# deevinandu/Distributed-Multi-Agent-SLAM-Swarm-Robotics-System

Measured on NVIDIA B200. Metric: beam_cell_updates_per_sec, higher is better.
Workload: dtype f64+u32

## Files before the change

### distributed-multi-agent-slam-swarm-robotics-system_b200/csrc/occgrid_tiled.cu

```cuda
#include "common.cuh"

namespace occ {

constexpr int kTT = 256;
constexpr int kChunkPk = 2048;
constexpr int kChunkMin = 256;
constexpr int kItemsPerCta = 3;
constexpr int kMaxWindowBytes = 100 * 1024;

struct TilePlanHeader {
    unsigned int n_items, n_active, total_records, work_counter, resolve_counter, overflow;
    unsigned int active_count;
    unsigned int pad;
};

__device__ __forceinline__ int home_tile(const Geom& g, const TileGeom& tg, double rx, double ry) {
    const double qx = cell_quotient(rx, g.ox, g.res), qy = cell_quotient(ry, g.oy, g.res);
    if (!quotient_in_range(qx) || !quotient_in_range(qy)) return -1;
    const int px = trunc_cell(qx) - g.win_x0 + tg.pad, py = trunc_cell(qy) - g.win_y0 + tg.pad;
    if (px < tg.pad - tg.reach || py < tg.pad - tg.reach || px >= tg.pad + g.win_w + tg.reach ||
        py >= tg.pad + g.win_h + tg.reach)
        return -1;
    return (py >> kTileShift) * tg.tiles_x + (px >> kTileShift);
}

constexpr int kPkPerCta = 2048;
constexpr int kSub = kPkPerCta / kTT;
constexpr int kHash = 4096;
constexpr unsigned int kEmpty = 0xffffffffu;
static_assert(kHash >= 2 * kPkPerCta, "hash table must stay at most half full");

__device__ __forceinline__ int hash_insert(unsigned int* keys, unsigned int tile) {
    unsigned int h = (tile * 2654435761u) >> 20;
    for (;;) {
        const unsigned int old = atomicCAS(&keys[h], kEmpty, tile);
        if (old == kEmpty || old == tile) return (int)h;
        h = (h + 1) & (kHash - 1);
    }
}

constexpr int kHashPerThread = kHash / kTT;

__device__ __forceinline__ void flush_tile_counts(const unsigned int* s_keys, const unsigned int* s_vals,
                                                  unsigned int* __restrict__ tile_count, unsigned int* __restrict__ active,
                                                  TilePlanHeader* __restrict__ hdr) {
    unsigned int key[kHashPerThread], old[kHashPerThread];
#pragma unroll
    for (int j = 0; j < kHashPerThread; ++j) {
        const int i = j * kTT + threadIdx.x;
        key[j] = s_keys[i];
        old[j] = 1u;
        if (key[j] != kEmpty) old[j] = atomicAdd(&tile_count[key[j]], s_vals[i]);
    }
#pragma unroll
    for (int j = 0; j < kHashPerThread; ++j)
        if (key[j] != kEmpty && old[j] == 0u) active[atomicAdd(&hdr->active_count, 1u)] = key[j];
}

__device__ __forceinline__ void reserve_tile_ranges(const unsigned int* s_keys, unsigned int* s_vals,
                                                    const unsigned int* __restrict__ tile_offset, unsigned int* __restrict__ tile_cursor) {
    unsigned int key[kHashPerThread], base[kHashPerThread], off[kHashPerThread];
#pragma unroll
    for (int j = 0; j < kHashPerThread; ++j) {
        const int i = j * kTT + threadIdx.x;
        key[j] = s_keys[i];
        base[j] = off[j] = 0u;
        if (key[j] != kEmpty) { off[j] = tile_offset[key[j]]; base[j] = atomicAdd(&tile_cursor[key[j]], s_vals[i]); }
    }
#pragma unroll
    for (int j = 0; j < kHashPerThread; ++j)
        if (key[j] != kEmpty) s_vals[j * kTT + threadIdx.x] = off[j] + base[j];
}

constexpr size_t kBinSmem = (size_t)kTT * kMaxRecStride + 2 * kHash * sizeof(unsigned int) + kPkPerCta * sizeof(unsigned short);
constexpr unsigned int kNoSlot = 0xffffu;

template <bool kMaps = false>
__global__ void __launch_bounds__(kTT)
k_home_bin(Geom g, TileGeom tg, const uint8_t* __restrict__ pkts, long long n, int stride,
           const int32_t* __restrict__ agent_idx, const double* __restrict__ drift,
           const double* __restrict__ agent_off, int n_agents,
           unsigned int* __restrict__ tile_count, PoseRec* __restrict__ recs, unsigned int* __restrict__ local_bins, uint2* __restrict__ runs,
           unsigned int* __restrict__ seg_count, unsigned int* __restrict__ active, TilePlanHeader* __restrict__ hdr,
           uint64_t* counters) {
    extern __shared__ __align__(16) uint8_t s_bin[];
    uint8_t* const s_rec = s_bin;
    unsigned int* const s_keys = reinterpret_cast<unsigned int*>(s_bin + kTT * kMaxRecStride);
    unsigned int* const s_vals = s_keys + kHash;
    unsigned short* const s_slot = reinterpret_cast<unsigned short*>(s_vals + kHash);
    __shared__ unsigned int s_wsum[kTT / 32];
    for (int i = threadIdx.x; i < kHash; i += kTT) { s_keys[i] = kEmpty; s_vals[i] = 0u; }
    unsigned long long c[OCCGRID_C_HITS + 1] = {};
    const long long cta_first = (long long)blockIdx.x * kPkPerCta;
    constexpr int kVec = (kTT * kMaxRecStride / 16 + kTT - 1) / kTT;
    uint4 pre[kVec];
    auto prefetch = [&](int sub) {
        const long long first = cta_first + (long long)sub * kTT;
        const long long left = n - first;
        const size_t bytes = left <= 0 ? 0 : (size_t)min((long long)kTT, left) * stride;
        const uint4* s4 = reinterpret_cast<const uint4*>(pkts + (size_t)first * stride);
#pragma unroll
        for (int j = 0; j < kVec; ++j) {
            const size_t i = (size_t)j * kTT + threadIdx.x;
            pre[j] = (i * 16 + 16 <= bytes) ? __ldg(s4 + i) : make_uint4(0u, 0u, 0u, 0u);
        }
    };
    const bool vec_ok = (reinterpret_cast<uintptr_t>(pkts) & 15) == 0 && ((kTT * stride) & 15) == 0;
    if (vec_ok) prefetch(0);
    for (int sub = 0; sub < kSub; ++sub) {
        const long long first = cta_first + (long long)sub * kTT;
        if (first >= n) break;
        const int count = (int)min((long long)kTT, n - first);
        __syncthreads();
        if (vec_ok) {
            const size_t bytes = (size_t)count * stride;
            uint4* d4 = reinterpret_cast<uint4*>(s_rec);
#pragma unroll
            for (int j = 0; j < kVec; ++j) {
                const size_t i = (size_t)j * kTT + threadIdx.x;
                if (i * 16 + 16 <= bytes) d4[i] = pre[j];
            }
            for (size_t i = (bytes / 16) * 16 + threadIdx.x; i < bytes; i += kTT) s_rec[i] = __ldg(pkts + (size_t)first * stride + i);
            if (sub + 1 < kSub) prefetch(sub + 1);
        } else {
            stage_records(pkts + (size_t)first * stride, (size_t)count * stride, s_rec);
        }
        __syncthreads();
        if ((int)threadIdx.x < count) {
            const long long k = first + threadIdx.x;
            double rx, ry, ryaw;
            float dist[4];
            c[OCCGRID_C_PACKETS] += 1;
            unsigned int slot = kNoSlot;
            int agent = 1;
            const int st = decode_packet(s_rec + threadIdx.x * stride, k, agent_idx, drift, agent_off, n_agents, &rx, &ry, &ryaw, dist,
                                         kMaps ? &agent : nullptr);
            if (st == PKT_DROPPED) c[OCCGRID_C_DROPPED] += 1;
            else if (st == PKT_BAD_POSE) c[OCCGRID_C_BAD_POSE] += 1;
            else {
                c[OCCGRID_C_ACCEPTED] += 1;
                c[OCCGRID_C_BEAMS] += 4;
#pragma unroll
                for (int s = 0; s < 4; ++s) {
                    const double d = (double)dist[s];
                    c[OCCGRID_C_HITS] += (OCC_MIN_DIST_M < d && d <= OCC_MAX_DIST_M) ? 1 : 0;
                }
                int tile = home_tile(g, tg, rx, ry);
                if (kMaps && tile >= 0) tile += (agent - 1) * tg.n_tiles;
                if (tile >= 0) {
                    slot = (unsigned int)hash_insert(s_keys, (unsigned int)tile);
                    atomicAdd(&s_vals[slot], 1u);
                    PoseRec r;
                    r.rx = rx; r.ry = ry; r.yaw = (float)ryaw;
                    r.d[0] = dist[0]; r.d[1] = dist[1]; r.d[2] = dist[2]; r.d[3] = dist[3];
                    r.k = (unsigned int)k;
                    r.tile = tile; r.pad = 0;
                    recs[k] = r;
                }
            }
            s_slot[sub * kTT + threadIdx.x] = (unsigned short)slot;
        }
    }
    __syncthreads();
    unsigned int key[kHashPerThread], rank[kHashPerThread];
#pragma unroll
    for (int j = 0; j < kHashPerThread; ++j) {
        const int i = j * kTT + threadIdx.x;
        key[j] = s_keys[i];
        rank[j] = 0u;
        if (key[j] != kEmpty) rank[j] = atomicAdd(&tile_count[key[j]], s_vals[i]);
    }
    const int lane = threadIdx.x & 31, warp = threadIdx.x >> 5;
    unsigned int mine = 0u;
#pragma unroll
    for (int j = 0; j < kHashPerThread; ++j) mine += key[j] != kEmpty ? s_vals[j * kTT + threadIdx.x] + 0x10000u : 0u;
    unsigned int inc = mine;
#pragma unroll
    for (int o = 1; o < 32; o <<= 1) { const unsigned int u = __shfl_up_sync(0xffffffffu, inc, o); if (lane >= o) inc += u; }
    if (lane == 31) s_wsum[warp] = inc;
    __syncthreads();
    unsigned int pos = inc - mine, n_local = 0u;
#pragma unroll
    for (int w = 0; w < kTT / 32; ++w) {
        pos += w < warp ? s_wsum[w] : 0u;
        n_local += s_wsum[w];
    }
    n_local &= 0xffffu;
    if (threadIdx.x == 0) seg_count[blockIdx.x] = n_local;
    const size_t seg0 = (size_t)blockIdx.x * kPkPerCta;
#pragma unroll
    for (int j = 0; j < kHashPerThread; ++j) {
        if (key[j] == kEmpty) continue;
        const int i = j * kTT + threadIdx.x;
        const unsigned int run = pos >> 16, begin = pos & 0xffffu;
        runs[seg0 + run] = make_uint2(key[j], rank[j] - begin);
        pos += s_vals[i] + 0x10000u;
        s_keys[i] = run;
        s_vals[i] = begin;
        if (rank[j] == 0u) active[atomicAdd(&hdr->active_count, 1u)] = key[j];
    }
    __syncthreads();
    unsigned int* const s_local = reinterpret_cast<unsigned int*>(s_rec);
    const int n_seg = (int)min((long long)kPkPerCta, n - (long long)seg0);
    for (int j = threadIdx.x; j < n_seg; j += kTT) {
        const unsigned int slot = s_slot[j];
        if (slot != kNoSlot) s_local[atomicAdd(&s_vals[slot], 1u)] = (s_keys[slot] << 16) | (unsigned int)j;
    }
    __syncthreads();
    for (unsigned int j = threadIdx.x; j < n_local; j += kTT) local_bins[seg0 + j] = s_local[j];
    __syncthreads();
    block_add_counters(c, reinterpret_cast<unsigned long long*>(s_rec), counters);
}

__global__ void __launch_bounds__(kTT)
k_place_runs(const unsigned int* __restrict__ local_bins, const uint2* __restrict__ runs, const unsigned int* __restrict__ seg_count,
             const unsigned int* __restrict__ tile_offset, const TilePlanHeader* __restrict__ hdr, unsigned int* __restrict__ bins) {
    if (hdr->overflow) return;
    const size_t seg0 = (size_t)blockIdx.x * kPkPerCta;
    const int n_local = (int)seg_count[blockIdx.x];
    unsigned int e[kSub], off[kSub];
    uint2 d[kSub];
#pragma unroll
    for (int sub = 0; sub < kSub; ++sub) {
        const int j = sub * kTT + threadIdx.x;
        e[sub] = j < n_local ? local_bins[seg0 + j] : kEmpty;
    }
#pragma unroll
    for (int sub = 0; sub < kSub; ++sub) d[sub] = e[sub] != kEmpty ? runs[seg0 + (e[sub] >> 16)] : make_uint2(0u, 0u);
#pragma unroll
    for (int sub = 0; sub < kSub; ++sub) off[sub] = e[sub] != kEmpty ? tile_offset[d[sub].x] : 0u;
#pragma unroll
    for (int sub = 0; sub < kSub; ++sub)
        if (e[sub] != kEmpty) bins[off[sub] + d[sub].y + (unsigned int)(sub * kTT + threadIdx.x)] = (unsigned int)(seg0 + (e[sub] & 0xffffu));
}

__device__ __forceinline__ int chunk_valid(const SegInfo& seg, long long chunk, long long* addr0) {
    const long long a0 = chunk * kSegChunk;
    *addr0 = a0;
    const unsigned int sg = (unsigned int)(a0 / seg.seg_cap);
    const unsigned int j0 = (unsigned int)(a0 - (long long)sg * seg.seg_cap);
    unsigned int cnt = seg.d_counts ? seg.d_counts[sg] : seg.host_count;
    if (cnt > seg.seg_cap) cnt = seg.seg_cap;
    return cnt > j0 ? (int)min((unsigned int)kSegChunk, cnt - j0) : 0;
}

__global__ void __launch_bounds__(kTT)
k_home_count_poses(Geom g, TileGeom tg, const PoseRec* __restrict__ recs, const int* __restrict__ in_tiles, SegInfo seg, long long n_chunks,
                   int tiles_in_records,
                   unsigned int* __restrict__ tile_count, int* __restrict__ tile_ids,
                   unsigned int* __restrict__ active, TilePlanHeader* __restrict__ hdr, uint64_t* counters) {
    __shared__ unsigned int s_keys[kHash];
    __shared__ unsigned int s_vals[kHash];
    __shared__ unsigned long long s_acc[(OCCGRID_C_HITS + 1) * 32];
    unsigned long long c[OCCGRID_C_HITS + 1] = {};
    for (long long chunk = blockIdx.x; chunk < n_chunks; chunk += gridDim.x) {
        long long addr0;
        const int valid = chunk_valid(seg, chunk, &addr0);
        if (valid == 0) continue;
        for (int i = threadIdx.x; i < kHash; i += kTT) { s_keys[i] = kEmpty; s_vals[i] = 0u; }
        __syncthreads();
        if (tiles_in_records) {
            int tl[kSub];
#pragma unroll
            for (int sub = 0; sub < kSub; ++sub) {
                const int j = sub * kTT + threadIdx.x;
                tl[sub] = -1;
                if (j < valid) tl[sub] = in_tiles ? in_tiles[addr0 + j] : recs[addr0 + j].tile;
            }
#pragma unroll
            for (int sub = 0; sub < kSub; ++sub) {
                const int j = sub * kTT + threadIdx.x;
                if (j >= valid) continue;
                int tile = tl[sub];
                if (tile >= tg.n_tiles) tile = -1;
                if (tile >= 0) atomicAdd(&s_vals[hash_insert(s_keys, (unsigned int)tile)], 1u);
                tile_ids[addr0 + j] = tile;
            }
        } else {
            for (int sub = 0; sub < kSub; ++sub) {
                const int j = sub * kTT + threadIdx.x;
                if (j >= valid) break;
                const long long k = addr0 + j;
                int tile = -1;
                const PoseRec r = recs[k];
                c[OCCGRID_C_PACKETS] += 1;
                if (!(isfinite(r.rx) && isfinite(r.ry) && isfinite(r.yaw))) c[OCCGRID_C_BAD_POSE] += 1;
                else {
                    c[OCCGRID_C_ACCEPTED] += 1;
                    c[OCCGRID_C_BEAMS] += 4;
#pragma unroll
                    for (int s2 = 0; s2 < 4; ++s2) {
                        const double dd = (double)r.d[s2];
                        c[OCCGRID_C_HITS] += (OCC_MIN_DIST_M < dd && dd <= OCC_MAX_DIST_M) ? 1 : 0;
                    }
                    tile = home_tile(g, tg, r.rx, r.ry);
                }
                if (tile >= 0) atomicAdd(&s_vals[hash_insert(s_keys, (unsigned int)tile)], 1u);
                tile_ids[k] = tile;
            }
        }
        __syncthreads();
        flush_tile_counts(s_keys, s_vals, tile_count, active, hdr);
        __syncthreads();
    }
    block_add_counters(c, s_acc, counters);
}

__global__ void __launch_bounds__(kTT)
k_home_scatter_segs(SegInfo seg, long long n_chunks, const int* __restrict__ tile_ids, const unsigned int* __restrict__ tile_offset,
                    unsigned int* __restrict__ tile_cursor, const TilePlanHeader* __restrict__ hdr, unsigned int* __restrict__ bins) {
    __shared__ unsigned int s_keys[kHash];
    __shared__ unsigned int s_vals[kHash];
    if (hdr->overflow) return;
    for (long long chunk = blockIdx.x; chunk < n_chunks; chunk += gridDim.x) {
        long long addr0;
        const int valid = chunk_valid(seg, chunk, &addr0);
        if (valid == 0) continue;
        for (int i = threadIdx.x; i < kHash; i += kTT) { s_keys[i] = kEmpty; s_vals[i] = 0u; }
        __syncthreads();
        unsigned int where[kSub];
        int tl[kSub];
#pragma unroll
        for (int sub = 0; sub < kSub; ++sub) {
            const int j = sub * kTT + threadIdx.x;
            tl[sub] = j < valid ? tile_ids[addr0 + j] : -1;
        }
#pragma unroll
        for (int sub = 0; sub < kSub; ++sub) {
            const int j = sub * kTT + threadIdx.x;
            where[sub] = kEmpty;
            if (j < valid) {
                const int tile = tl[sub];
                if (tile >= 0) {
                    const int h = hash_insert(s_keys, (unsigned int)tile);
                    where[sub] = ((unsigned int)h << 16) | atomicAdd(&s_vals[h], 1u);
                }
            }
        }
        __syncthreads();
        reserve_tile_ranges(s_keys, s_vals, tile_offset, tile_cursor);
        __syncthreads();
#pragma unroll
        for (int sub = 0; sub < kSub; ++sub)
            if (where[sub] != kEmpty)
                bins[s_vals[where[sub] >> 16] + (where[sub] & 0xffffu)] = (unsigned int)(addr0 + sub * kTT + threadIdx.x);
        __syncthreads();
    }
}

__global__ void __launch_bounds__(1024)
k_tile_plan(unsigned int* __restrict__ tile_count, unsigned int* __restrict__ tile_offset,
            unsigned int* __restrict__ tile_cursor, uint4* __restrict__ items, unsigned int max_items,
            const unsigned int* __restrict__ active, unsigned long long max_records, TilePlanHeader* __restrict__ hdr,
            uint64_t* counters, unsigned int target_items) {
    __shared__ unsigned int s_warp[2][33];
    __shared__ unsigned int s_carry[2];
    __shared__ unsigned int s_total;
    if (threadIdx.x < 2) s_carry[threadIdx.x] = 0;
    if (threadIdx.x == 0) s_total = 0;
    __syncthreads();
    const int n_active = (int)hdr->active_count;
    const int lane = threadIdx.x & 31, warp = threadIdx.x >> 5;
    {
        unsigned int mine = 0;
        for (int i = threadIdx.x; i < n_active; i += blockDim.x) mine += tile_count[active[i]];
#pragma unroll
        for (int o = 16; o > 0; o >>= 1) mine += __shfl_xor_sync(0xffffffffu, mine, o);
        if (lane == 0 && mine) atomicAdd(&s_total, mine);
    }
    __syncthreads();
    unsigned int chunk_pk = (s_total / target_items + kChunkMin) / kChunkMin * kChunkMin;
    chunk_pk = chunk_pk > (unsigned int)kChunkPk ? (unsigned int)kChunkPk : chunk_pk;
    for (int start = 0; start < n_active; start += blockDim.x) {
        const int i = start + threadIdx.x;
        const unsigned int t = i < n_active ? active[i] : 0u;
        const unsigned int cnt = i < n_active ? tile_count[t] : 0u;
        unsigned int v[2] = {cnt, (cnt + chunk_pk - 1) / chunk_pk};
        unsigned int ex[2];
#pragma unroll
        for (int j = 0; j < 2; ++j) {
            unsigned int inc = v[j];
#pragma unroll
            for (int o = 1; o < 32; o <<= 1) { unsigned int u = __shfl_up_sync(0xffffffffu, inc, o); if (lane >= o) inc += u; }
            if (lane == 31) s_warp[j][warp] = inc;
            ex[j] = inc - v[j];
        }
        __syncthreads();
        if (warp < 2) {
            unsigned int w = s_warp[warp][lane], winc = w;
#pragma unroll
            for (int o = 1; o < 32; o <<= 1) { unsigned int u = __shfl_up_sync(0xffffffffu, winc, o); if (lane >= o) winc += u; }
            s_warp[warp][lane] = winc - w;
            if (lane == 31) s_warp[warp][32] = winc;
        }
        __syncthreads();
        const unsigned int off = s_carry[0] + s_warp[0][warp] + ex[0];
        const unsigned int item0 = s_carry[1] + s_warp[1][warp] + ex[1];
        if (i < n_active) {
            tile_offset[t] = off;
            tile_cursor[t] = 0u;
            tile_count[t] = 0u;
            for (unsigned int j = 0; j < v[1]; ++j) {
                const unsigned int b = off + j * chunk_pk;
                const unsigned int e = min(off + cnt, b + chunk_pk);
                if (item0 + j < max_items) items[item0 + j] = make_uint4(t, b, e, 0u);
            }
        }
        __syncthreads();
        if (threadIdx.x < 2) s_carry[threadIdx.x] += s_warp[threadIdx.x][32];
        __syncthreads();
    }
    if (threadIdx.x == 0) {
        TilePlanHeader h;
        h.total_records = s_carry[0];
        h.n_items = s_carry[1];
        h.n_active = (unsigned int)n_active;
        h.work_counter = 0;
        h.resolve_counter = 0;
        h.active_count = 0;
        h.overflow = (s_carry[0] > max_records || s_carry[1] > max_items) ? 1u : 0u;
        if (h.overflow) { h.n_items = 0; h.n_active = 0; }
        h.pad = 0;
        *hdr = h;
        if (counters) atomicAdd(reinterpret_cast<unsigned long long*>(counters) + OCCGRID_C_RECORDS, (unsigned long long)s_carry[0]);
    }
}

__device__ __noinline__ void draw_beam_smem(unsigned int* __restrict__ s_win, int side, int pitch, int x, int y,
                                               int ddx, int ddy, unsigned int free_stamp, bool hit, bool skip_first) {
    const int dx = abs(ddx), dy = abs(ddy);
    int err = dx - dy;
    const int n = max(dx, dy);
    const unsigned int us = (unsigned int)side;
    if ((unsigned int)x < us && (unsigned int)y < us && (unsigned int)(x + ddx) < us && (unsigned int)(y + ddy) < us) {
        const int sxo = ddx > 0 ? 1 : -1;
        const int syo = ddy > 0 ? pitch : -pitch;
        const bool xmajor = dx >= dy;
        const int dmaj = xmajor ? dx : dy, dmin = xmajor ? dy : dx;
        const int step_maj = xmajor ? sxo : syo;
        const int step_both = sxo + syo;
        const int e_minor = dmaj - dmin;
        int E = dmaj - dmin;
        int off = y * pitch + x;
        int i = 0;
        if (skip_first) {
            if (n == 0) return;
            const bool minor = 2 * E < dmaj;
            off += minor ? step_both : step_maj;
            E += minor ? e_minor : -dmin;
            i = 1;
        }
        for (; i < n; ++i) {
            atomicMax(&s_win[off], free_stamp);
            const bool minor = 2 * E < dmaj;
            off += minor ? step_both : step_maj;
            E += minor ? e_minor : -dmin;
        }
        if (hit) atomicMax(&s_win[off], free_stamp | 1u);
        return;
    }
    const int sx = ddx > 0 ? 1 : -1, sy = ddy > 0 ? 1 : -1;
    for (int i = 0; i < n; ++i) {
        if (!(i == 0 && skip_first) && (unsigned int)x < us && (unsigned int)y < us) atomicMax(&s_win[y * pitch + x], free_stamp);
        const int e2 = 2 * err;
        if (e2 > -dy) { err -= dy; x += sx; }
        if (e2 < dx)  { err += dx; y += sy; }
    }
    if (hit && !(n == 0 && skip_first) && (unsigned int)x < us && (unsigned int)y < us) atomicMax(&s_win[y * pitch + x], free_stamp | 1u);
}

__device__ __noinline__ void count_beam_smem(unsigned int* __restrict__ s_win, int side, int pitch, int x, int y,
                                                int ddx, int ddy, bool hit) {
    const int dx = abs(ddx), dy = abs(ddy);
    const int n = max(dx, dy);
    const unsigned int us = (unsigned int)side;
    if ((unsigned int)x < us && (unsigned int)y < us && (unsigned int)(x + ddx) < us && (unsigned int)(y + ddy) < us) {
        const int sxo = ddx > 0 ? 1 : -1;
        const int syo = ddy > 0 ? pitch : -pitch;
        const bool xmajor = dx >= dy;
        const int dmaj = xmajor ? dx : dy, dmin = xmajor ? dy : dx;
        const int step_maj = xmajor ? sxo : syo;
        const int step_both = sxo + syo;
        const int e_minor = dmaj - dmin;
        int E = dmaj - dmin;
        int off = y * pitch + x;
        for (int i = 0; i < n; ++i) {
            atomicAdd(&s_win[off], 1u);
            const bool minor = 2 * E < dmaj;
            off += minor ? step_both : step_maj;
            E += minor ? e_minor : -dmin;
        }
        if (hit) atomicAdd(&s_win[off], 0x10000u);
        return;
    }
    int err = dx - dy;
    const int sx = ddx > 0 ? 1 : -1, sy = ddy > 0 ? 1 : -1;
    for (int i = 0; i < n; ++i) {
        if ((unsigned int)x < us && (unsigned int)y < us) atomicAdd(&s_win[y * pitch + x], 1u);
        const int e2 = 2 * err;
        if (e2 > -dy) { err -= dy; x += sx; }
        if (e2 < dx)  { err += dx; y += sy; }
    }
    if (hit && (unsigned int)x < us && (unsigned int)y < us) atomicAdd(&s_win[y * pitch + x], 0x10000u);
}



constexpr int kMaskMaxLen = 32;
constexpr int kMaskEntries = (kMaskMaxLen + 1) * (kMaskMaxLen + 2) / 2;

__device__ __forceinline__ unsigned int walk_mask_of(int dmaj, int dmin) {
    unsigned int m = 0u;
    int E = dmaj - dmin;
    for (int i = 0; i < dmaj; ++i) {
        const bool minor = 2 * E < dmaj;
        m |= (minor ? 1u : 0u) << i;
        E += minor ? (dmaj - dmin) : -dmin;
    }
    return m;
}

__device__ __forceinline__ void build_walk_masks(unsigned int* s_mask) {
    for (int e = threadIdx.x; e < kMaskEntries; e += blockDim.x) {
        int dmaj = 0;
        while ((dmaj + 1) * (dmaj + 2) / 2 <= e) ++dmaj;
        s_mask[e] = walk_mask_of(dmaj, e - dmaj * (dmaj + 1) / 2);
    }
}

template <bool kAdd>
__device__ __forceinline__ void smem_red(unsigned int addr, unsigned int v) {
    if (kAdd) asm volatile("red.shared.add.u32 [%0], %1;" ::"r"(addr), "r"(v) : "memory");
    else      asm volatile("red.shared.max.u32 [%0], %1;" ::"r"(addr), "r"(v) : "memory");
}

template <bool kAdd>
__device__ __forceinline__ void walk_beam_masked(unsigned int win, int pitch, int x, int y, int ddx, int ddy,
                                                 unsigned int v_free, bool hit, bool skip_first, const unsigned int* s_mask) {
    const int dx = abs(ddx), dy = abs(ddy);
    const bool xmajor = dx >= dy;
    const int dmaj = xmajor ? dx : dy, dmin = xmajor ? dy : dx;
    const int sx4 = ddx > 0 ? 4 : -4;
    const int sy4 = (ddy > 0 ? pitch : -pitch) * 4;
    const int step_maj = xmajor ? sx4 : sy4, step_min = xmajor ? sy4 : sx4;
    unsigned int mask = s_mask[dmaj * (dmaj + 1) / 2 + dmin];
    unsigned int a = win + (unsigned int)(y * pitch + x) * 4u;
    const unsigned int a_end = a + (unsigned int)((ddy * pitch + ddx) * 4);
    int rem = dmaj;
    if (rem > 0) {
        if (!skip_first) smem_red<kAdd>(a, v_free);
        a += step_maj + ((mask & 1u) ? step_min : 0);
        mask >>= 1;
        --rem;
    }
    while (rem >= 8) {
#pragma unroll
        for (int j = 0; j < 8; ++j) {
            smem_red<kAdd>(a, v_free);
            a += step_maj + ((mask & (1u << j)) ? step_min : 0);
        }
        mask >>= 8;
        rem -= 8;
    }
    if (rem >= 4) {
#pragma unroll
        for (int j = 0; j < 4; ++j) {
            smem_red<kAdd>(a, v_free);
            a += step_maj + ((mask & (1u << j)) ? step_min : 0);
        }
        mask >>= 4;
        rem -= 4;
    }
    for (; rem > 0; --rem) {
        smem_red<kAdd>(a, v_free);
        a += step_maj + ((mask & 1u) ? step_min : 0);
        mask >>= 1;
    }
// ... 395 lines not shown
        for (int ly = ly_lo + part * (kTT / 32) + warp; ly < ly_hi; ly += kResolveSplit * (kTT / 32)) {
            const size_t row = (size_t)(wy0 + ly) * g.win_w + wx0;
            for (int lx = lx_lo + lane; lx < lx_hi; lx += 32) {
                const unsigned int s = plane[row + lx];
                if (s) {
                    map_grid[row + lx] = (s & 1u) ? OCCGRID_CELL_OCCUPIED : OCCGRID_CELL_FREE;
                    plane[row + lx] = 0u;
                }
            }
        }
    }
}


static int g_raycast_cta_cap = 0;
void set_raycast_cta_cap(int cap) { g_raycast_cta_cap = cap < 0 ? 0 : cap; }

struct TiledLayout {
    size_t off_stamps, off_count, off_offset, off_cursor, off_active, off_hdr, off_items, off_ids, off_bins, off_local, off_runs,
        off_segs, off_recs, total;
    unsigned long long max_records;
    unsigned int max_items;
};

static TiledLayout tiled_layout(const occgrid_geom* geom, int64_t max_records, bool packets, int n_maps = 1) {
    TiledLayout L;
    const TileGeom tg = tile_geom(geom);
    const size_t n_keys = (size_t)n_maps * tg.n_tiles;
    L.max_records = (unsigned long long)max_records;
    unsigned long long items = L.max_records / kChunkMin + (unsigned long long)n_keys + 1;
    if (items > L.max_records + 1) items = L.max_records + 1;
    L.max_items = (unsigned int)items;
    size_t o = 0;
    L.off_stamps = o; o += align_up((size_t)geom->win_w * geom->win_h * 4 * (size_t)n_maps, 256);
    L.off_count = o;  o += align_up((n_keys + 1) * 4, 256);
    L.off_offset = o; o += align_up((n_keys + 1) * 4, 256);
    L.off_cursor = o; o += align_up((n_keys + 1) * 4, 256);
    L.off_active = o; o += align_up((n_keys + 1) * 4, 256);
    L.off_hdr = o;    o += 256;
    L.off_items = o;  o += align_up((size_t)L.max_items * sizeof(uint4), 256);
    L.off_ids = o;    o += packets ? 0 : align_up((size_t)L.max_records * sizeof(int), 256);
    L.off_bins = o;   o += align_up((size_t)L.max_records * sizeof(unsigned int), 256);
    L.off_local = o;  o += packets ? align_up((size_t)L.max_records * sizeof(unsigned int), 256) : 0;
    L.off_runs = o;   o += packets ? align_up((size_t)L.max_records * sizeof(uint2), 256) : 0;
    L.off_segs = o;   o += packets ? align_up((size_t)(L.max_records + kPkPerCta - 1) / kPkPerCta * sizeof(unsigned int), 256) : 0;
    L.off_recs = o;   o += packets ? align_up((size_t)L.max_records * sizeof(PoseRec), 256) : 0;
    L.total = o;
    return L;
}

bool tiled_supported(const occgrid_geom* geom, int n_maps) {
    const TileGeom tg = tile_geom(geom);
    return (size_t)tg.win_side * tg.pitch * 4 <= (size_t)kMaxWindowBytes && (long long)n_maps * tg.n_tiles <= (1ll << 24);
}

size_t tiled_workspace_bytes(const occgrid_geom* geom, int n_maps, int64_t max_packets) {
    return tiled_layout(geom, max_packets < 1 ? 1 : max_packets, true, n_maps).total;
}

size_t tiled_band_workspace_bytes(const occgrid_geom* geom, int n_segs, int64_t seg_cap) {
    return tiled_layout(geom, (int64_t)n_segs * seg_cap, false).total;
}

struct TiledPtrs {
    unsigned int *stamps, *tile_count, *tile_offset, *tile_cursor, *active, *bins, *local_bins, *seg_count;
    TilePlanHeader* hdr;
    uint4* items;
    int* tile_ids;
    uint2* runs;
    PoseRec* recs;
};

static TiledPtrs tiled_ptrs(const TiledLayout& L, void* d_ws) {
    char* ws = reinterpret_cast<char*>(d_ws);
    TiledPtrs p;
    p.stamps = reinterpret_cast<unsigned int*>(ws + L.off_stamps);
    p.tile_count = reinterpret_cast<unsigned int*>(ws + L.off_count);
    p.tile_offset = reinterpret_cast<unsigned int*>(ws + L.off_offset);
    p.tile_cursor = reinterpret_cast<unsigned int*>(ws + L.off_cursor);
    p.active = reinterpret_cast<unsigned int*>(ws + L.off_active);
    p.hdr = reinterpret_cast<TilePlanHeader*>(ws + L.off_hdr);
    p.items = reinterpret_cast<uint4*>(ws + L.off_items);
    p.bins = reinterpret_cast<unsigned int*>(ws + L.off_bins);
    p.tile_ids = reinterpret_cast<int*>(ws + L.off_ids);
    p.local_bins = reinterpret_cast<unsigned int*>(ws + L.off_local);
    p.runs = reinterpret_cast<uint2*>(ws + L.off_runs);
    p.seg_count = reinterpret_cast<unsigned int*>(ws + L.off_segs);
    p.recs = reinterpret_cast<PoseRec*>(ws + L.off_recs);
    return p;
}

static size_t raycast_smem(const TileGeom& tg, bool route) {
    size_t b = (size_t)tg.win_side * tg.pitch * 4;
    const size_t r = (size_t)kRouteItemPk * 2 * sizeof(PoseRec);
    const size_t raw = (size_t)kRouteItemPk * kMaxRecStride;
    if (route) b = b > r ? b : r;
    if (route) b = b > raw ? b : raw;
    return b;
}

template <bool kCounts, bool kRoute, bool kMaps = false>
static int launch_raycast(const Geom& g, const TileGeom& tg, const TiledPtrs& P, const PoseRec* recs, int ordinals_in_records,
                          unsigned int* plane, uint64_t* d_counters, int have_items, const RouteJob& job, cudaStream_t st) {
    const size_t smem = raycast_smem(tg, kRoute);
    static thread_local size_t configured = 0;
    if (smem > configured) {
        OCC_CUDA_TRY(cudaFuncSetAttribute(k_home_raycast<kCounts, kRoute, kMaps>, cudaFuncAttributeMaxDynamicSharedMemorySize, (int)smem));
        configured = smem;
    }
    int ctas_per_sm = 1;
    if (cudaOccupancyMaxActiveBlocksPerMultiprocessor(&ctas_per_sm, k_home_raycast<kCounts, kRoute, kMaps>, kTT, smem) != cudaSuccess || ctas_per_sm < 1)
        ctas_per_sm = 1;
    if (g_raycast_cta_cap > 0 && ctas_per_sm > g_raycast_cta_cap) ctas_per_sm = g_raycast_cta_cap;
    ProfileScope ps(K_TILE_RAYCAST, st);
    k_home_raycast<kCounts, kRoute, kMaps><<<device_sm_count() * ctas_per_sm, kTT, smem, st>>>(g, tg, P.items, P.hdr, P.bins, recs,
                                                                                               ordinals_in_records, plane, d_counters,
                                                                                               have_items, job);
    return OCCGRID_OK;
}

static unsigned int plan_target_items() { return (unsigned int)device_sm_count() * 3u * (unsigned int)kItemsPerCta; }

static int grid_chunks(long long n_chunks) {
    long long b = n_chunks < 1 ? 1 : n_chunks;
    const long long cap = (long long)device_sm_count() * 8;
    return (int)(b < cap ? b : cap);
}

int integrate_tiled(const occgrid_geom* geom, const PacketBatch& batch, const PoseRec* d_poses, int ordinals_in_records, Output kind,
                    void* d_out, void* d_ws, size_t ws_bytes, uint64_t* d_counters, cudaStream_t st) {
    const int64_t n = batch.n;
    const bool maps = kind == Output::kAgentMaps;
    const TiledLayout L = tiled_layout(geom, n, d_poses == nullptr, maps ? batch.n_agents : 1);
    if (ws_bytes < L.total) {
        set_last_error("workspace %zu B < %zu B needed by TILED for %lld records", ws_bytes, L.total, (long long)n);
        return OCCGRID_E_WORKSPACE;
    }
    const TiledPtrs P = tiled_ptrs(L, d_ws);
    const PoseRec* recs = d_poses ? d_poses : P.recs;
    const Geom g = to_geom(geom);
    const TileGeom tg = tile_geom(geom);
    const unsigned int blocks = (unsigned int)((n + kPkPerCta - 1) / kPkPerCta);
    SegInfo seg;
    seg.n_segs = 1; seg.seg_cap = (unsigned int)align_up((size_t)n, kSegChunk); seg.d_counts = nullptr; seg.host_count = (unsigned int)n;
    const long long n_chunks = (n + kSegChunk - 1) / kSegChunk;
    {
        ProfileScope ps(K_TILE_COUNT, st);
        if (d_poses) {
            k_home_count_poses<<<grid_chunks(n_chunks), kTT, 0, st>>>(g, tg, d_poses, nullptr, seg, n_chunks, 0, P.tile_count, P.tile_ids, P.active,
                                                                      P.hdr, d_counters);
        } else {
            const auto bin = maps ? k_home_bin<true> : k_home_bin<false>;
            OCC_CUDA_TRY(cudaFuncSetAttribute(bin, cudaFuncAttributeMaxDynamicSharedMemorySize, (int)kBinSmem));
            bin<<<blocks, kTT, kBinSmem, st>>>(g, tg, batch.pkts, n, batch.stride, batch.agent_idx, batch.drift, batch.agent_off, batch.n_agents,
                                               P.tile_count, P.recs, P.local_bins, P.runs, P.seg_count, P.active, P.hdr, d_counters);
        }
    }
    {
        ProfileScope ps(K_TILE_SCAN, st);
        k_tile_plan<<<1, 1024, 0, st>>>(P.tile_count, P.tile_offset, P.tile_cursor, P.items, L.max_items, P.active, L.max_records, P.hdr,
                                        d_counters, plan_target_items());
    }
    {
        ProfileScope ps(K_TILE_SCATTER, st);
        if (d_poses) k_home_scatter_segs<<<grid_chunks(n_chunks), kTT, 0, st>>>(seg, n_chunks, P.tile_ids, P.tile_offset, P.tile_cursor, P.hdr, P.bins);
        else         k_place_runs<<<blocks, kTT, 0, st>>>(P.local_bins, P.runs, P.seg_count, P.tile_offset, P.hdr, P.bins);
    }
    RouteJob none = {};
    unsigned int* const plane = kind == Output::kCounts ? reinterpret_cast<unsigned int*>(d_out) : P.stamps;
    if (kind == Output::kCounts) launch_raycast<true, false>(g, tg, P, recs, ordinals_in_records, plane, d_counters, 1, none, st);
    else if (maps)               launch_raycast<false, false, true>(g, tg, P, recs, ordinals_in_records, plane, d_counters, 1, none, st);
    else                         launch_raycast<false, false>(g, tg, P, recs, ordinals_in_records, plane, d_counters, 1, none, st);
    if (kind != Output::kCounts) {
        ProfileScope ps(K_TILE_RESOLVE, st);
        const auto resolve = maps ? k_home_resolve<true> : k_home_resolve<false>;
        resolve<<<device_sm_count() * 8, kTT, 0, st>>>(g, tg, P.active, P.hdr, P.stamps, reinterpret_cast<int8_t*>(d_out));
    }
    OCC_CUDA_TRY(cudaGetLastError());
    return OCCGRID_OK;
}

int tiled_prepare_poses(const occgrid_geom* geom, const PoseRec* d_recs, const int* d_tiles, const SegInfo& seg, int tiles_in_records,
                        void* d_ws, size_t ws_bytes, uint64_t* d_counters, cudaStream_t st) {
    const int64_t max_records = (int64_t)seg.n_segs * seg.seg_cap;
    const TiledLayout L = tiled_layout(geom, max_records, false);
    if (ws_bytes < L.total) {
        set_last_error("workspace %zu B < %zu B needed by the band step for %lld record addresses", ws_bytes, L.total, (long long)max_records);
        return OCCGRID_E_WORKSPACE;
    }
    const TiledPtrs P = tiled_ptrs(L, d_ws);
    const Geom g = to_geom(geom);
    const TileGeom tg = tile_geom(geom);
    const long long n_chunks = max_records / kSegChunk;
    {
        ProfileScope ps(K_TILE_COUNT, st);
        k_home_count_poses<<<grid_chunks(n_chunks), kTT, 0, st>>>(g, tg, d_recs, d_tiles, seg, n_chunks, tiles_in_records, P.tile_count, P.tile_ids,
                                                                  P.active, P.hdr, d_counters);
    }
    {
        ProfileScope ps(K_TILE_SCAN, st);
        k_tile_plan<<<1, 1024, 0, st>>>(P.tile_count, P.tile_offset, P.tile_cursor, P.items, L.max_items, P.active, L.max_records, P.hdr,
                                        d_counters, plan_target_items());
    }
    {
        ProfileScope ps(K_TILE_SCATTER, st);
        k_home_scatter_segs<<<grid_chunks(n_chunks), kTT, 0, st>>>(seg, n_chunks, P.tile_ids, P.tile_offset, P.tile_cursor, P.hdr, P.bins);
    }
    OCC_CUDA_TRY(cudaGetLastError());
    return OCCGRID_OK;
}

int tiled_raycast_route(const occgrid_geom* geom, const PoseRec* d_recs, int have_items, const RouteJob* job,
                        int8_t* d_grid, void* d_ws, size_t ws_bytes, int64_t max_records, uint64_t* d_counters, cudaStream_t st,
                        cudaEvent_t after_fused) {
    const TiledLayout L = tiled_layout(geom, max_records, false);
    if (ws_bytes < L.total) { set_last_error("workspace too small for the band step"); return OCCGRID_E_WORKSPACE; }
    const TiledPtrs P = tiled_ptrs(L, d_ws);
    const Geom g = to_geom(geom);
    const TileGeom tg = tile_geom(geom);
    if (!have_items) {
        OCC_CUDA_TRY(cudaMemsetAsync(P.hdr, 0, sizeof(TilePlanHeader), st));
    }
    if (job) {
        launch_raycast<false, true>(g, tg, P, d_recs, 1, P.stamps, d_counters, have_items, *job, st);
    } else {
        RouteJob none = {};
        launch_raycast<false, false>(g, tg, P, d_recs, 1, P.stamps, d_counters, have_items, none, st);
    }
    if (after_fused) OCC_CUDA_TRY(cudaEventRecord(after_fused, st));
    if (have_items) {
        ProfileScope ps(K_TILE_RESOLVE, st);
        k_home_resolve<false><<<device_sm_count() * 8, kTT, 0, st>>>(g, tg, P.active, P.hdr, P.stamps, d_grid);
    }
    OCC_CUDA_TRY(cudaGetLastError());
    return OCCGRID_OK;
}

}
```

Baseline: 677.3 billion.

## Restructure home-bin staging with cp.async rounds and inline packet decode; rework tile plan scan

The binning kernel now stages two-thread-widths of packets per round with cp.async double-buffered prefetch, decodes the wire fields inline with funnel shifts instead of calling decode_packet, caches agent offsets in shared memory, and uses 32-bit counters. Home-tile computation uses a fast reciprocal-multiply quotient and falls back to exact division only near cell boundaries. The single-block tile plan kernel is rewritten to process four tiles per thread with one packed 64-bit block scan, replacing two separate scans and extra barriers. It also sets a max-shared carveout. Risks include subtle decode or rounding divergence from the original path, and the prefetch overlapping less because the wait occurs right before use.

```diff
diff --git a/distributed-multi-agent-slam-swarm-robotics-system_b200/csrc/occgrid_tiled.cu b/distributed-multi-agent-slam-swarm-robotics-system_b200/csrc/occgrid_tiled.cu
--- a/distributed-multi-agent-slam-swarm-robotics-system_b200/csrc/occgrid_tiled.cu
+++ b/distributed-multi-agent-slam-swarm-robotics-system_b200/csrc/occgrid_tiled.cu
@@ -14,8 +14,7 @@
     unsigned int pad;
 };
 
-__device__ __forceinline__ int home_tile(const Geom& g, const TileGeom& tg, double rx, double ry) {
-    const double qx = cell_quotient(rx, g.ox, g.res), qy = cell_quotient(ry, g.oy, g.res);
+__device__ __forceinline__ int home_tile_of(const Geom& g, const TileGeom& tg, double qx, double qy) {
     if (!quotient_in_range(qx) || !quotient_in_range(qy)) return -1;
     const int px = trunc_cell(qx) - g.win_x0 + tg.pad, py = trunc_cell(qy) - g.win_y0 + tg.pad;
     if (px < tg.pad - tg.reach || py < tg.pad - tg.reach || px >= tg.pad + g.win_w + tg.reach ||
@@ -24,6 +23,18 @@
     return (py >> kTileShift) * tg.tiles_x + (px >> kTileShift);
 }
 
+__device__ __forceinline__ int home_tile(const Geom& g, const TileGeom& tg, double rx, double ry) {
+    return home_tile_of(g, tg, cell_quotient(rx, g.ox, g.res), cell_quotient(ry, g.oy, g.res));
+}
+
+__device__ __forceinline__ int home_tile_screened(const Geom& g, const TileGeom& tg, double rx, double ry, double ryaw) {
+    double qx = OCC_DMUL(OCC_DADD(rx, -g.ox), g.inv_res);
+    double qy = OCC_DMUL(OCC_DADD(ry, -g.oy), g.inv_res);
+    if (near_cell_boundary(qx, screening_tolerance(rx, g.ox, ryaw, g.inv_res))) qx = cell_quotient(rx, g.ox, g.res);
+    if (near_cell_boundary(qy, screening_tolerance(ry, g.oy, ryaw, g.inv_res))) qy = cell_quotient(ry, g.oy, g.res);
+    return home_tile_of(g, tg, qx, qy);
+}
+
 constexpr int kPkPerCta = 2048;
 constexpr int kSub = kPkPerCta / kTT;
 constexpr int kHash = 4096;
@@ -72,8 +83,38 @@
         if (key[j] != kEmpty) s_vals[j * kTT + threadIdx.x] = off[j] + base[j];
 }
 
-constexpr size_t kBinSmem = (size_t)kTT * kMaxRecStride + 2 * kHash * sizeof(unsigned int) + kPkPerCta * sizeof(unsigned short);
+constexpr int kBinRound = 2 * kTT;
+constexpr int kBinRounds = kPkPerCta / kBinRound;
+constexpr int kBinAgentCap = 256;
+constexpr size_t kBinSmem = (size_t)kBinRound * kMaxRecStride + 2 * kHash * sizeof(unsigned int) + kPkPerCta * sizeof(unsigned short);
 constexpr unsigned int kNoSlot = 0xffffu;
+static_assert(kPkPerCta % kBinRound == 0, "a segment is a whole number of rounds");
+
+__device__ __forceinline__ void cp_async_16(void* smem, const void* gmem, int src_bytes) {
+    asm volatile("cp.async.cg.shared.global [%0], [%1], 16, %2;\n" ::"r"((unsigned int)__cvta_generic_to_shared(smem)),
+                 "l"(__cvta_generic_to_global(gmem)), "r"(src_bytes) : "memory");
+}
+__device__ __forceinline__ void cp_async_wait_all() { asm volatile("cp.async.wait_all;\n" ::: "memory"); }
+
+struct WireFields {
+    unsigned int b0, head;
+    float f[7];
+};
+
+__device__ __forceinline__ WireFields read_wire_fields(const uint8_t* s_rec, int base) {
+    const unsigned int* w = reinterpret_cast<const unsigned int*>(s_rec) + ((base + 1) >> 2);
+    const unsigned int sh = (unsigned int)((base + 1) & 3) * 8u;
+    unsigned int u[11];
+#pragma unroll
+    for (int m = 0; m < 11; ++m) u[m] = m == 5 ? 0u : w[m];
+    WireFields r;
+    r.b0 = s_rec[base];
+    r.head = __funnelshift_r(u[0], u[1], sh);
+    constexpr int kWord[7] = {1, 2, 3, 6, 7, 8, 9};
+#pragma unroll
+    for (int i = 0; i < 7; ++i) r.f[i] = __uint_as_float(__funnelshift_r(u[kWord[i]], u[kWord[i] + 1], sh));
+    return r;
+}
 
 template <bool kMaps = false>
 __global__ void __launch_bounds__(kTT)
@@ -85,80 +126,92 @@
            uint64_t* counters) {
     extern __shared__ __align__(16) uint8_t s_bin[];
     uint8_t* const s_rec = s_bin;
-    unsigned int* const s_keys = reinterpret_cast<unsigned int*>(s_bin + kTT * kMaxRecStride);
+    unsigned int* const s_keys = reinterpret_cast<unsigned int*>(s_bin + kBinRound * kMaxRecStride);
     unsigned int* const s_vals = s_keys + kHash;
     unsigned short* const s_slot = reinterpret_cast<unsigned short*>(s_vals + kHash);
     __shared__ unsigned int s_wsum[kTT / 32];
+    __shared__ double s_agent_off[2 * (kBinAgentCap + 1)];
     for (int i = threadIdx.x; i < kHash; i += kTT) { s_keys[i] = kEmpty; s_vals[i] = 0u; }
-    unsigned long long c[OCCGRID_C_HITS + 1] = {};
+    const bool agents_shared = n_agents <= kBinAgentCap;
+    if (agents_shared)
+        for (int i = threadIdx.x; i < 2 * (n_agents + 1); i += kTT) s_agent_off[i] = agent_off[i];
+    const double* const aoff = agents_shared ? s_agent_off : agent_off;
+    unsigned int c[OCCGRID_C_HITS + 1] = {};
     const long long cta_first = (long long)blockIdx.x * kPkPerCta;
-    constexpr int kVec = (kTT * kMaxRecStride / 16 + kTT - 1) / kTT;
-    uint4 pre[kVec];
-    auto prefetch = [&](int sub) {
-        const long long first = cta_first + (long long)sub * kTT;
-        const long long left = n - first;
-        const size_t bytes = left <= 0 ? 0 : (size_t)min((long long)kTT, left) * stride;
-        const uint4* s4 = reinterpret_cast<const uint4*>(pkts + (size_t)first * stride);
-#pragma unroll
-        for (int j = 0; j < kVec; ++j) {
-            const size_t i = (size_t)j * kTT + threadIdx.x;
-            pre[j] = (i * 16 + 16 <= bytes) ? __ldg(s4 + i) : make_uint4(0u, 0u, 0u, 0u);
+    const bool async_ok = (reinterpret_cast<uintptr_t>(pkts) & 15) == 0;
+    auto stage = [&](int round) {
+        const long long first = cta_first + (long long)round * kBinRound;
+        const int bytes = (int)min((long long)kBinRound, n - first) * stride;
+        const uint8_t* src = pkts + (size_t)first * stride;
+        if (async_ok) {
+            for (int i = threadIdx.x * 16; i < bytes; i += kTT * 16) cp_async_16(s_rec + i, src + i, min(16, bytes - i));
+        } else {
+            stage_records(src, (size_t)bytes, s_rec);
         }
     };
-    const bool vec_ok = (reinterpret_cast<uintptr_t>(pkts) & 15) == 0 && ((kTT * stride) & 15) == 0;
-    if (vec_ok) prefetch(0);
-    for (int sub = 0; sub < kSub; ++sub) {
-        const long long first = cta_first + (long long)sub * kTT;
+    stage(0);
+    for (int round = 0; round < kBinRounds; ++round) {
+        const long long first = cta_first + (long long)round * kBinRound;
         if (first >= n) break;
-        const int count = (int)min((long long)kTT, n - first);
-        __syncthreads();
-        if (vec_ok) {
-            const size_t bytes = (size_t)count * stride;
-            uint4* d4 = reinterpret_cast<uint4*>(s_rec);
-#pragma unroll
-            for (int j = 0; j < kVec; ++j) {
-                const size_t i = (size_t)j * kTT + threadIdx.x;
-                if (i * 16 + 16 <= bytes) d4[i] = pre[j];
-            }
-            for (size_t i = (bytes / 16) * 16 + threadIdx.x; i < bytes; i += kTT) s_rec[i] = __ldg(pkts + (size_t)first * stride + i);
-            if (sub + 1 < kSub) prefetch(sub + 1);
-        } else {
-            stage_records(pkts + (size_t)first * stride, (size_t)count * stride, s_rec);
-        }
-        __syncthreads();
-        if ((int)threadIdx.x < count) {
-            const long long k = first + threadIdx.x;
-            double rx, ry, ryaw;
-            float dist[4];
+        const int count = (int)min((long long)kBinRound, n - first);
+        cp_async_wait_all();
+        __syncthreads();
+        WireFields w[2];
+        int agent[2];
+#pragma unroll
+        for (int q = 0; q < 2; ++q) {
+            const int j = q * kTT + threadIdx.x;
+            if (j < count) {
+                w[q] = read_wire_fields(s_rec, j * stride);
+                agent[q] = agent_idx ? agent_idx[first + j] : (int)(w[q].head >> 24);
+            }
+        }
+        __syncthreads();
+        if (round + 1 < kBinRounds && first + kBinRound < n) stage(round + 1);
+#pragma unroll
+        for (int q = 0; q < 2; ++q) {
+            const int j = q * kTT + threadIdx.x;
+            if (j >= count) continue;
+            const long long k = first + j;
             c[OCCGRID_C_PACKETS] += 1;
             unsigned int slot = kNoSlot;
-            int agent = 1;
-            const int st = decode_packet(s_rec + threadIdx.x * stride, k, agent_idx, drift, agent_off, n_agents, &rx, &ry, &ryaw, dist,
-                                         kMaps ? &agent : nullptr);
-            if (st == PKT_DROPPED) c[OCCGRID_C_DROPPED] += 1;
-            else if (st == PKT_BAD_POSE) c[OCCGRID_C_BAD_POSE] += 1;
-            else {
-                c[OCCGRID_C_ACCEPTED] += 1;
-                c[OCCGRID_C_BEAMS] += 4;
-#pragma unroll
-                for (int s = 0; s < 4; ++s) {
-                    const double d = (double)dist[s];
-                    c[OCCGRID_C_HITS] += (OCC_MIN_DIST_M < d && d <= OCC_MAX_DIST_M) ? 1 : 0;
+            const bool magic = w[q].b0 == 'Q' && (w[q].head & 0xffffffu) == ('S' | ('R' << 8) | ('L' << 16));
+            const int a = agent[q];
+            if (!magic || a < 1 || a > n_agents) {
+                c[OCCGRID_C_DROPPED] += 1;
+            } else {
+                double rx = OCC_DADD((double)w[q].f[0], aoff[2 * a + 0]);
+                double ry = OCC_DADD((double)w[q].f[1], aoff[2 * a + 1]);
+                const double ryaw = (double)w[q].f[2];
+                if (drift) {
+                    rx = OCC_DADD(rx, drift[2 * k + 0]);
+                    ry = OCC_DADD(ry, drift[2 * k + 1]);
                 }
-                int tile = home_tile(g, tg, rx, ry);
-                if (kMaps && tile >= 0) tile += (agent - 1) * tg.n_tiles;
-                if (tile >= 0) {
-                    slot = (unsigned int)hash_insert(s_keys, (unsigned int)tile);
-                    atomicAdd(&s_vals[slot], 1u);
-                    PoseRec r;
-                    r.rx = rx; r.ry = ry; r.yaw = (float)ryaw;
-                    r.d[0] = dist[0]; r.d[1] = dist[1]; r.d[2] = dist[2]; r.d[3] = dist[3];
-                    r.k = (unsigned int)k;
-                    r.tile = tile; r.pad = 0;
-                    recs[k] = r;
+                if (!(isfinite(rx) && isfinite(ry) && isfinite(ryaw))) {
+                    c[OCCGRID_C_BAD_POSE] += 1;
+                } else {
+                    c[OCCGRID_C_ACCEPTED] += 1;
+                    c[OCCGRID_C_BEAMS] += 4;
+#pragma unroll
+                    for (int s = 0; s < 4; ++s) {
+                        const double d = (double)w[q].f[3 + s];
+                        c[OCCGRID_C_HITS] += (OCC_MIN_DIST_M < d && d <= OCC_MAX_DIST_M) ? 1 : 0;
+                    }
+                    int tile = home_tile_screened(g, tg, rx, ry, ryaw);
+                    if (kMaps && tile >= 0) tile += (a - 1) * tg.n_tiles;
+                    if (tile >= 0) {
+                        slot = (unsigned int)hash_insert(s_keys, (unsigned int)tile);
+                        atomicAdd(&s_vals[slot], 1u);
+                        PoseRec r;
+                        r.rx = rx; r.ry = ry; r.yaw = w[q].f[2];
+                        r.d[0] = w[q].f[3]; r.d[1] = w[q].f[4]; r.d[2] = w[q].f[5]; r.d[3] = w[q].f[6];
+                        r.k = (unsigned int)k;
+                        r.tile = tile; r.pad = 0;
+                        recs[k] = r;
+                    }
                 }
             }
-            s_slot[sub * kTT + threadIdx.x] = (unsigned short)slot;
+            s_slot[round * kBinRound + j] = (unsigned short)slot;
         }
     }
     __syncthreads();
@@ -209,7 +262,10 @@
     __syncthreads();
     for (unsigned int j = threadIdx.x; j < n_local; j += kTT) local_bins[seg0 + j] = s_local[j];
     __syncthreads();
-    block_add_counters(c, reinterpret_cast<unsigned long long*>(s_rec), counters);
+    unsigned long long c64[OCCGRID_C_HITS + 1];
+#pragma unroll
+    for (int i = 0; i <= OCCGRID_C_HITS; ++i) c64[i] = c[i];
+    block_add_counters(c64, reinterpret_cast<unsigned long long*>(s_rec), counters);
 }
 
 __global__ void __launch_bounds__(kTT)
@@ -348,81 +404,82 @@
     }
 }
 
-__global__ void __launch_bounds__(1024)
+constexpr int kPlanThreads = 1024;
+constexpr int kPlanPer = 4;
+__global__ void __launch_bounds__(kPlanThreads)
 k_tile_plan(unsigned int* __restrict__ tile_count, unsigned int* __restrict__ tile_offset,
             unsigned int* __restrict__ tile_cursor, uint4* __restrict__ items, unsigned int max_items,
             const unsigned int* __restrict__ active, unsigned long long max_records, TilePlanHeader* __restrict__ hdr,
             uint64_t* counters, unsigned int target_items) {
-    __shared__ unsigned int s_warp[2][33];
-    __shared__ unsigned int s_carry[2];
-    __shared__ unsigned int s_total;
-    if (threadIdx.x < 2) s_carry[threadIdx.x] = 0;
-    if (threadIdx.x == 0) s_total = 0;
-    __syncthreads();
+    __shared__ unsigned int s_part[kPlanThreads / 32];
+    __shared__ unsigned long long s_scan[33];
     const int n_active = (int)hdr->active_count;
     const int lane = threadIdx.x & 31, warp = threadIdx.x >> 5;
-    {
-        unsigned int mine = 0;
-        for (int i = threadIdx.x; i < n_active; i += blockDim.x) mine += tile_count[active[i]];
-#pragma unroll
-        for (int o = 16; o > 0; o >>= 1) mine += __shfl_xor_sync(0xffffffffu, mine, o);
-        if (lane == 0 && mine) atomicAdd(&s_total, mine);
-    }
+    constexpr int kPass = kPlanThreads * kPlanPer;
+    unsigned int t[kPlanPer], cnt[kPlanPer];
+    auto load = [&](int i0) {
+#pragma unroll
+        for (int j = 0; j < kPlanPer; ++j) t[j] = i0 + j < n_active ? active[i0 + j] : 0u;
+#pragma unroll
+        for (int j = 0; j < kPlanPer; ++j) cnt[j] = i0 + j < n_active ? tile_count[t[j]] : 0u;
+    };
+    load((int)threadIdx.x * kPlanPer);
+    unsigned int mine = 0;
+#pragma unroll
+    for (int j = 0; j < kPlanPer; ++j) mine += cnt[j];
+    for (int i = kPass + threadIdx.x; i < n_active; i += kPlanThreads) mine += tile_count[active[i]];
+#pragma unroll
+    for (int o = 16; o > 0; o >>= 1) mine += __shfl_xor_sync(0xffffffffu, mine, o);
+    if (lane == 0) s_part[warp] = mine;
     __syncthreads();
-    unsigned int chunk_pk = (s_total / target_items + kChunkMin) / kChunkMin * kChunkMin;
+    unsigned int total = 0;
+#pragma unroll
+    for (int w = 0; w < kPlanThreads / 32; ++w) total += s_part[w];
+    unsigned int chunk_pk = (total / target_items + kChunkMin) / kChunkMin * kChunkMin;
     chunk_pk = chunk_pk > (unsigned int)kChunkPk ? (unsigned int)kChunkPk : chunk_pk;
-    for (int start = 0; start < n_active; start += blockDim.x) {
-        const int i = start + threadIdx.x;
-        const unsigned int t = i < n_active ? active[i] : 0u;
-        const unsigned int cnt = i < n_active ? tile_count[t] : 0u;
-        unsigned int v[2] = {cnt, (cnt + chunk_pk - 1) / chunk_pk};
-        unsigned int ex[2];
-#pragma unroll
-        for (int j = 0; j < 2; ++j) {
-            unsigned int inc = v[j];
-#pragma unroll
-            for (int o = 1; o < 32; o <<= 1) { unsigned int u = __shfl_up_sync(0xffffffffu, inc, o); if (lane >= o) inc += u; }
-            if (lane == 31) s_warp[j][warp] = inc;
-            ex[j] = inc - v[j];
-        }
-        __syncthreads();
-        if (warp < 2) {
-            unsigned int w = s_warp[warp][lane], winc = w;
-#pragma unroll
-            for (int o = 1; o < 32; o <<= 1) { unsigned int u = __shfl_up_sync(0xffffffffu, winc, o); if (lane >= o) winc += u; }
-            s_warp[warp][lane] = winc - w;
-            if (lane == 31) s_warp[warp][32] = winc;
-        }
-        __syncthreads();
-        const unsigned int off = s_carry[0] + s_warp[0][warp] + ex[0];
-        const unsigned int item0 = s_carry[1] + s_warp[1][warp] + ex[1];
-        if (i < n_active) {
-            tile_offset[t] = off;
-            tile_cursor[t] = 0u;
-            tile_count[t] = 0u;
-            for (unsigned int j = 0; j < v[1]; ++j) {
-                const unsigned int b = off + j * chunk_pk;
-                const unsigned int e = min(off + cnt, b + chunk_pk);
-                if (item0 + j < max_items) items[item0 + j] = make_uint4(t, b, e, 0u);
-            }
-        }
-        __syncthreads();
-        if (threadIdx.x < 2) s_carry[threadIdx.x] += s_warp[threadIdx.x][32];
-        __syncthreads();
+    unsigned long long carry = 0;
+    for (int start = 0; start < n_active; start += kPass) {
+        const int i0 = start + (int)threadIdx.x * kPlanPer;
+        if (start > 0) load(i0);
+        unsigned long long v[kPlanPer], sum = 0;
+#pragma unroll
+        for (int j = 0; j < kPlanPer; ++j) {
+            v[j] = ((unsigned long long)((cnt[j] + chunk_pk - 1) / chunk_pk) << 32) | cnt[j];
+            sum += v[j];
+        }
+        unsigned long long pass_total;
+        unsigned long long run = carry + block_exclusive_scan(sum, s_scan, &pass_total);
+#pragma unroll
+        for (int j = 0; j < kPlanPer; ++j) {
+            if (i0 + j < n_active) {
+                const unsigned int off = (unsigned int)run, item0 = (unsigned int)(run >> 32), n_it = (unsigned int)(v[j] >> 32);
+                tile_offset[t[j]] = off;
+                tile_cursor[t[j]] = 0u;
+                tile_count[t[j]] = 0u;
+                for (unsigned int k = 0; k < n_it; ++k) {
+                    const unsigned int b = off + k * chunk_pk;
+                    const unsigned int e = min(off + cnt[j], b + chunk_pk);
+                    if (item0 + k < max_items) items[item0 + k] = make_uint4(t[j], b, e, 0u);
+                }
+            }
+            run += v[j];
+        }
+        carry += pass_total;
     }
     if (threadIdx.x == 0) {
+        const unsigned int n_records = (unsigned int)carry, n_items = (unsigned int)(carry >> 32);
         TilePlanHeader h;
-        h.total_records = s_carry[0];
-        h.n_items = s_carry[1];
+        h.total_records = n_records;
+        h.n_items = n_items;
         h.n_active = (unsigned int)n_active;
         h.work_counter = 0;
         h.resolve_counter = 0;
         h.active_count = 0;
-        h.overflow = (s_carry[0] > max_records || s_carry[1] > max_items) ? 1u : 0u;
+        h.overflow = (n_records > max_records || n_items > max_items) ? 1u : 0u;
         if (h.overflow) { h.n_items = 0; h.n_active = 0; }
         h.pad = 0;
         *hdr = h;
-        if (counters) atomicAdd(reinterpret_cast<unsigned long long*>(counters) + OCCGRID_C_RECORDS, (unsigned long long)s_carry[0]);
+        if (counters) atomicAdd(reinterpret_cast<unsigned long long*>(counters) + OCCGRID_C_RECORDS, (unsigned long long)n_records);
     }
 }
 
@@ -1124,13 +1181,14 @@
         } else {
             const auto bin = maps ? k_home_bin<true> : k_home_bin<false>;
             OCC_CUDA_TRY(cudaFuncSetAttribute(bin, cudaFuncAttributeMaxDynamicSharedMemorySize, (int)kBinSmem));
+            OCC_CUDA_TRY(cudaFuncSetAttribute(bin, cudaFuncAttributePreferredSharedMemoryCarveout, (int)cudaSharedmemCarveoutMaxShared));
             bin<<<blocks, kTT, kBinSmem, st>>>(g, tg, batch.pkts, n, batch.stride, batch.agent_idx, batch.drift, batch.agent_off, batch.n_agents,
                                                P.tile_count, P.recs, P.local_bins, P.runs, P.seg_count, P.active, P.hdr, d_counters);
         }
     }
     {
         ProfileScope ps(K_TILE_SCAN, st);
-        k_tile_plan<<<1, 1024, 0, st>>>(P.tile_count, P.tile_offset, P.tile_cursor, P.items, L.max_items, P.active, L.max_records, P.hdr,
+        k_tile_plan<<<1, kPlanThreads, 0, st>>>(P.tile_count, P.tile_offset, P.tile_cursor, P.items, L.max_items, P.active, L.max_records, P.hdr,
                                         d_counters, plan_target_items());
     }
     {
@@ -1171,7 +1229,7 @@
     }
     {
         ProfileScope ps(K_TILE_SCAN, st);
-        k_tile_plan<<<1, 1024, 0, st>>>(P.tile_count, P.tile_offset, P.tile_cursor, P.items, L.max_items, P.active, L.max_records, P.hdr,
+        k_tile_plan<<<1, kPlanThreads, 0, st>>>(P.tile_count, P.tile_offset, P.tile_cursor, P.items, L.max_items, P.active, L.max_records, P.hdr,
                                         d_counters, plan_target_items());
     }
     {
```

Result: faster. 694.6 billion, median of 6 (+2.6%).
